# Yan-Xia/Text2Loc

Measured on AMD Instinct MI355X. Metric: coarse-retrieval queries/sec over 11k-cell DB, embed_dim=256; top-1/3/5 recall parity, higher is better.
Workload: dtype f16; 1 GPU; KITTI360Pose-sized val DB: N=11259 cells x D=256 resident in HBM, Q=4096 precomputed text embeddings per step, top-10 (float64-exact ids); n_cells=11259, embed_dim=256, top_k=10, parallelism=single-gpu, layout=one resident DB, two launches per step (scan, re-rank)

## Files before the change

include/t2l.h:

```cpp
#ifndef T2L_H_
#define T2L_H_

#include <stdint.h>

#ifdef __cplusplus
extern "C" {
#endif

#define T2L_ABI_VERSION 2
#define T2L_EMBED_DIM 256
#define T2L_OBJECT_SIZE 28
#define T2L_MAX_LOSS_BATCH 1024
#define T2L_MAX_TOPK 26

enum {
  T2L_OK = 0,
  T2L_EINVAL = -1,
  T2L_ESTATE = -2,
  T2L_EHIP = -3,
  T2L_ENOMEM = -4
};

typedef struct t2l_ctx t2l_ctx;

// ... 65 lines not shown
                       double* out_score, void* stream);

int t2l_merge_topk(t2l_ctx* ctx, const int32_t* idx, const double* score, int32_t parts, int32_t n_queries,
                   int32_t k, int32_t* out_idx, double* out_score, void* stream);

int t2l_pack_pairs(t2l_ctx* ctx, const int32_t* idx, const double* score, int32_t n_queries, int32_t k, double* pairs,
                   void* stream);
int t2l_merge_pairs(t2l_ctx* ctx, const double* pairs, int32_t parts, int32_t n_queries, int32_t k, int32_t* out_idx,
                    double* out_score, void* stream);
int t2l_merge_gathered(t2l_ctx* ctx, const void* blocks, int64_t block_bytes, int64_t score_offset, int32_t parts,
                       int32_t n_queries, int32_t k, int32_t* out_idx, double* out_score, void* stream);

int t2l_search_fallbacks(t2l_ctx* ctx, int32_t* out_count);
int t2l_search_rescored(t2l_ctx* ctx, int32_t* out_count);
int t2l_search_counters(t2l_ctx* ctx, int32_t* out8);

int t2l_contrastive_loss(t2l_ctx* ctx, const float* anchor, const float* positive, int32_t batch,
                         float temperature, float* loss, float* grad_anchor, float* grad_positive,
                         void* stream);

int t2l_text_head_load_weights(t2l_ctx* ctx, const t2l_weight_desc* w, int32_t n, const char* prefix);
int t2l_text_head_load_weights_heads(t2l_ctx* ctx, const t2l_weight_desc* w, int32_t n, const char* prefix, int32_t inter_num_heads);
int t2l_text_head(t2l_ctx* ctx, const float* hidden, int32_t n_sentences, int32_t n_tokens, float* out, int32_t* overflow,
                  void* stream);
int t2l_text_inter(t2l_ctx* ctx, const float* sent, int32_t n_descriptions, int32_t n_sentences_per, float* out, int32_t* overflow,
                   void* stream);

int t2l_fine_load_weights(t2l_ctx* ctx, const t2l_weight_desc* w, int32_t n, const t2l_model_config* cfg);

int t2l_fine_encode_objects(t2l_ctx* ctx, const t2l_packed_cells* in, float* out_desc, void* stream);
// ... 60 lines not shown
```

text2loc_amd/csrc/capi.hip:

```cpp
#include <limits.h>
#include <string.h>

#include "t2l_internal.h"

namespace t2l {

int fail(t2l_ctx* ctx, int code, const std::string& msg) {
  if (ctx) ctx->err = msg;
  return code;
}

void event_begin(t2l_ctx* ctx, const char* name, hipStream_t s) {
  if (!ctx->profile_events) return;
  EventRing& e = ctx->events[name];
  if (e.a.empty()) {
    e.a.resize(kEventRing);
    e.b.resize(kEventRing);
    for (int i = 0; i < kEventRing; ++i) {
      (void)hipEventCreate(&e.a[i]);
      (void)hipEventCreate(&e.b[i]);
    }
  }
  e.open = (e.calls++ % ctx->profile_events) == 0;
  if (e.open) (void)hipEventRecord(e.a[e.head], s);
// ... 280 lines not shown
}

int t2l_merge_gathered(t2l_ctx* ctx, const void* blocks, int64_t block_bytes, int64_t score_offset, int32_t parts, int32_t n_queries,
                       int32_t k, int32_t* out_idx, double* out_score, void* stream) {
  if (!ctx) return T2L_EINVAL;
  if (parts < 1 || n_queries < 0 || k < 1 || k > T2L_MAX_TOPK)
    return fail(ctx, T2L_EINVAL, "t2l_merge_gathered: bad parts / n_queries / k");
  if (n_queries == 0) return T2L_OK;
  if (!blocks || !out_idx) return fail(ctx, T2L_EINVAL, "t2l_merge_gathered: null buffer");
  if (reinterpret_cast<uintptr_t>(blocks) % 8)
    return fail(ctx, T2L_EINVAL, "t2l_merge_gathered: blocks must start on an 8-byte boundary");
  T2L_HIP(ctx, hipSetDevice(ctx->device));
  return merge_gathered_impl(ctx, blocks, block_bytes, score_offset, parts, n_queries, k, out_idx, out_score, (hipStream_t)stream);
}

static hipError_t read_counters(t2l_ctx* ctx, int32_t* out8) {
  if (ctx->last_search_small) {
    for (int i = 0; i < 8; ++i) out8[i] = 0;
    return hipSuccess;
  }
  hipError_t e = hipMemcpy(out8, ctx->fb_count, 8 * sizeof(int32_t), hipMemcpyDeviceToHost);
  if (e != hipSuccess || ctx->n_lanes <= 1) return e;
  for (int i = 0; i < 8; ++i) out8[i] = 0;
  for (int l = 0; l < ctx->n_lanes; ++l) {
    if (!ctx->lanes[l].ready) continue;
    int32_t c[8];
    if ((e = hipMemcpy(c, ctx->lanes[l].fb_count, sizeof(c), hipMemcpyDeviceToHost)) != hipSuccess) return e;
    for (int i = 0; i < 8; ++i) out8[i] += c[i];
  }
  return hipSuccess;
}

int t2l_search_fallbacks(t2l_ctx* ctx, int32_t* out_count) {
  if (!ctx || !out_count) return T2L_EINVAL;
  T2L_HIP(ctx, hipSetDevice(ctx->device));
  T2L_HIP(ctx, hipDeviceSynchronize());
  int32_t c[8];
  T2L_HIP(ctx, read_counters(ctx, c));
  *out_count = c[kCntExactScan] + (c[kCntExactServed] - c[kCntExactUncert]);
  return T2L_OK;
}

#ifdef T2L_STAMPS
int t2l_debug_stamps(t2l_ctx* ctx, long long* out24) {
  T2L_HIP(ctx, hipDeviceSynchronize());
  T2L_HIP(ctx, hipMemcpy(out24, ctx->fb_count + 16, 24 * sizeof(long long), hipMemcpyDeviceToHost));
  const long long init[8] = {0, 0, 0, 0, LLONG_MAX, 0, LLONG_MAX, 0};
  T2L_HIP(ctx, hipMemcpy(ctx->fb_count + 16, init, sizeof(init), hipMemcpyHostToDevice));
  return T2L_OK;
}
#endif

int t2l_search_counters(t2l_ctx* ctx, int32_t* out8) {
  if (!ctx || !out8) return T2L_EINVAL;
  T2L_HIP(ctx, hipSetDevice(ctx->device));
  T2L_HIP(ctx, hipDeviceSynchronize());
  T2L_HIP(ctx, read_counters(ctx, out8));
  return T2L_OK;
}

int t2l_search_rescored(t2l_ctx* ctx, int32_t* out_count) {
  if (!ctx || !out_count) return T2L_EINVAL;
  T2L_HIP(ctx, hipSetDevice(ctx->device));
  T2L_HIP(ctx, hipDeviceSynchronize());
  int32_t c[8];
  T2L_HIP(ctx, read_counters(ctx, c));
  *out_count = c[kCntRescored];
  return T2L_OK;
}

int t2l_contrastive_loss(t2l_ctx* ctx, const float* anchor, const float* positive, int32_t batch, float temperature,
                         float* loss, float* grad_anchor, float* grad_positive, void* stream) {
// ... 227 lines not shown
    ctx->knobs.wide_repair = (int)value;
  } else if (!strcmp(name, "search_tile_sel")) {
    ctx->knobs.search_tile_sel = value != 0;
  } else if (!strcmp(name, "search_epilogue")) {
    if (value != 0 && value != 1) return fail(ctx, T2L_EINVAL, "search_epilogue: 0 (round 6's epilogue and record layout) or 1 (default)");
    ctx->knobs.search_epilogue = (int)value;
  } else if (!strcmp(name, "search_rerank_form")) {
#ifdef T2L_RERANK_PARTS
    if (value == 2 || value == 3) {
      ctx->knobs.rerank_form = (int)value;
      return T2L_OK;
    }
#endif
    if (value != 0 && value != 1) return fail(ctx, T2L_EINVAL, "search_rerank_form: 0 (round 7's re-rank of merged records) or 1 (default: row-local merge, one gather round trip)");
    ctx->knobs.rerank_form = (int)value;
  } else if (!strcmp(name, "search_pair_ll")) {
    if (value != 5 && value != 6) return fail(ctx, T2L_EINVAL, "search_pair_ll must be 5 or 6");
    ctx->knobs.pair_ll = (int)value;
  } else if (!strcmp(name, "train_gemm_block")) {
    if (value != 0 && value != 32 && value != 64) return fail(ctx, T2L_EINVAL, "train_gemm_block must be 0 (auto), 32 or 64");
    ctx->train_gemm_block = (int)value;
  } else if (!strcmp(name, "train_bf16")) {
    if (value != 0 && value != 1 && value != 2) return fail(ctx, T2L_EINVAL, "train_bf16: 0 (f32 MFMA), 1 (bf16 operands) or 2 (split-bf16, three products)");
    ctx->train_bf16 = (int)value;
  } else if (!strcmp(name, "train_keep_adam_state")) {
    ctx->train_keep_adam = value != 0;
  } else if (!strcmp(name, "profile_rerank")) {
    ctx->knobs.profile_rerank = value != 0;
  } else if (!strcmp(name, "stats_reset")) {
    for (auto& kv : ctx->events) {
// ... 81 lines not shown
```

text2loc_amd/csrc/search.hip:

```cpp
#include <float.h>
#include <limits.h>

#include <type_traits>
#include <utility>

#include "t2l_internal.h"
#include "search_dev.h"

namespace t2l {

__device__ __forceinline__ void reset_counts(int32_t* fb_count, int32_t* fb_prev, int zero_counts, int tid) {
  if (zero_counts && tid < kCntCleared) {
    fb_count[kReportBase + tid] = fb_prev[tid];
    fb_prev[tid] = 0;
  }
  if (!zero_counts && tid == 0) {
    fb_count[kCntDeferredSegs] += fb_count[kCntDeferred];
    fb_count[kCntDeferred] = fb_count[kCntExactUncert] = 0;
  }
}


__global__ __launch_bounds__(256) void split_db_kernel(const float* __restrict__ db, uint4* __restrict__ out, int rows) {
  const int gid = blockIdx.x * 256 + threadIdx.x;
// ... 251 lines not shown
  const float* q;
  int Q, K, parts, code_bits;
  const float* cand;
  int row_offset;
  float eps_rel;
  const float* db_norm_max;
  int half_mode;
  int32_t* out_idx;
  double* out_score;
  int32_t* flags;
  int32_t* fb_count;
  float eps_rel_probe, pinf;
  int n_rows, defer, wide_cap;
  int rec6;
  int slot_bits = 0;
};

#ifndef T2L_SEL_RD
#define T2L_SEL_RD 2
#endif
template <int LL, int NS, bool MERGE = false, int SEL = 0>
__global__ __launch_bounds__(512, 1) void scanp_kernel(const uint4* __restrict__ dbt, int n_rows, int n_tiles, int code_bits,
                                                       const float* __restrict__ q, int Q, int nsplit,
                                                       float* __restrict__ cand, int32_t* __restrict__ fb_count, int32_t* __restrict__ fb_prev,
                                                       int zero_counts, float pinf, unsigned long long* __restrict__ span,
                                                       unsigned span_seq, int xcd_qgroups, int slot_bits) {
  static_assert(NS == 4, "the step loop below is unrolled for a ring of 4 slots");
  constexpr bool EPI = SEL == 1;
  static_assert(!MERGE || LL == 6, "the in-workgroup list merge is written for lists of 6");
  static_assert(!SEL || MERGE, "the tile-local selection's dropped-bound leaves through the merged record's bound");
// ... 336 lines not shown
    put_list(qrow1, w.ls1);
  }
  if (span && threadIdx.x == 0) {
    const unsigned long long t1 = __builtin_amdgcn_s_memrealtime(), tag = (unsigned long long)span_seq << 40, tm = (1ull << 40) - 1;
    *reinterpret_cast<ulonglong2*>(span + 2 * blockIdx.x) = make_ulonglong2(tag | (wg_t0 & tm), tag | (t1 & tm));
  }
  T2L_STAMP(3);
}

template <int NW>
struct WgExactSharedN {
  double score[NW][32];
  int row[NW][32];
};
typedef WgExactSharedN<4> WgExactShared;

__device__ __forceinline__ void top32_insert(double& ts, int& tr, double cd, int cr, int lane) {
  {
    const unsigned long long b31 = __double_as_longlong(ts);
    const double s31 = __longlong_as_double(((unsigned long long)__builtin_amdgcn_readlane((unsigned)(b31 >> 32), 31) << 32) |
                                            (unsigned)__builtin_amdgcn_readlane((unsigned)b31, 31));
    const int r31 = __builtin_amdgcn_readlane(tr, 31);
    if (s31 > cd || (s31 == cd && r31 <= cr)) return;
  }
  if (__ballot(lane < 32 && tr == cr) != 0ull) return;
  const unsigned long long ahead = __ballot(lane < 32 && (ts > cd || (ts == cd && tr < cr)));
  const int pos = __popcll(ahead);
  if (pos >= 32) return;
  const double up_s = __shfl_up(ts, 1);
  const int up_r = __shfl_up(tr, 1);
  if (lane == pos) {
    ts = cd;
    tr = cr;
  } else if (lane > pos && lane < 32) {
    ts = up_s;
    tr = up_r;
  }
}

template <int NW = 4>
__device__ __forceinline__ void wg_exact_scan(const float* __restrict__ db, int n_rows, const float* __restrict__ qrow, int K,
                                              int row_offset, int32_t* __restrict__ out_idx, double* __restrict__ out_score,
                                              WgExactSharedN<NW>& sh) {
  const int lane = threadIdx.x & 63, wave = threadIdx.x >> 6;
  const int seg = lane & 15, grp = lane >> 4;
  double qd[16];
  {
    const float4* qp = reinterpret_cast<const float4*>(qrow) + seg;
#pragma unroll
    for (int i = 0; i < 4; ++i) {
      const float4 v = qp[16 * i];
      qd[4 * i] = (double)v.x;
      qd[4 * i + 1] = (double)v.y;
      qd[4 * i + 2] = (double)v.z;
      qd[4 * i + 3] = (double)v.w;
    }
  }
  double my_s = -__builtin_inf();
  int my_r = INT_MAX;
  const int n_groups = (n_rows + 3) / 4;
  for (int g = wave; g < n_groups; g += NW) {
    const int row = 4 * g + grp;
    const float4* rp = reinterpret_cast<const float4*>(db + (size_t)min(row, n_rows - 1) * kD) + seg;
    double d0 = 0.0, d1 = 0.0;
#pragma unroll
    for (int i = 0; i < 4; ++i) {
      const float4 rv = rp[16 * i];
      d0 += (double)rv.x * qd[4 * i];
      d1 += (double)rv.y * qd[4 * i + 1];
      d0 += (double)rv.z * qd[4 * i + 2];
      d1 += (double)rv.w * qd[4 * i + 3];
    }
    const double d = row16_sum_f64(d0 + d1);
#pragma unroll
    for (int c = 0; c < 4; ++c) {
      const double cd = __shfl(d, 16 * c);
      const int cr = 4 * g + c;
      if (cr >= n_rows) break;
      const unsigned long long ahead = __ballot(lane < 32 && (my_s > cd || (my_s == cd && my_r < cr)));
      const int pos = __popcll(ahead);
      if (pos >= 32) continue;
      const double up_s = __shfl_up(my_s, 1);
      const int up_r = __shfl_up(my_r, 1);
      if (lane == pos) {
        my_s = cd;
        my_r = cr;
      } else if (lane > pos && lane < 32) {
        my_s = up_s;
        my_r = up_r;
      }
    }
  }
  if (lane < 32) {
    sh.score[wave][lane] = my_s;
    sh.row[wave][lane] = my_r;
  }
  __syncthreads();
  if (wave == 0) {
    constexpr int PER = NW / 2, TOT = 32 * NW;
    double sv[PER];
    int rv[PER], kv[PER];
#pragma unroll
    for (int e = 0; e < PER; ++e) {
      sv[e] = (&sh.score[0][0])[64 * e + lane];
      rv[e] = (&sh.row[0][0])[64 * e + lane];
      kv[e] = 0;
    }
    for (int o = 0; o < TOT; ++o) {
      const double os = (&sh.score[0][0])[o];
      const int orow = (&sh.row[0][0])[o];
#pragma unroll
      for (int e = 0; e < PER; ++e) kv[e] += (os > sv[e] || (os == sv[e] && orow < rv[e])) ? 1 : 0;
    }
    if (lane < K) {
      out_idx[lane] = -1;
      if (out_score) out_score[lane] = -__builtin_inf();
    }
#pragma unroll
    for (int e = 0; e < PER; ++e)
      if (rv[e] != INT_MAX && kv[e] < K) {
        out_idx[kv[e]] = rv[e] + row_offset;
        if (out_score) out_score[kv[e]] = sv[e];
      }
  }
  __syncthreads();
}


__device__ __forceinline__ void publish_report(int32_t* fb_count, int32_t* host_stat, int seq) {
  if (host_stat && seq > 0) {
    const int32_t* prev = fb_count + kReportBase;
    host_stat[kStatFlagged] = prev[kCntStatMode] == 2 ? prev[kCntProbe] : prev[kCntUnsettled];
    host_stat[kStatTotal] = prev[kCntQ];
    host_stat[kStatExact] = prev[kCntExactScan] + prev[kCntDeferred] + prev[kCntDeferredSegs];
    host_stat[kStatMode] = prev[kCntStatMode];
    host_stat[kStatRescored] = prev[kCntStatMode] == 2 ? prev[kCntProbe] : prev[kCntRescored];
    __hip_atomic_store(&host_stat[kStatSeq], seq, __ATOMIC_RELEASE, __HIP_MEMORY_SCOPE_SYSTEM);
  }
}

#ifdef T2L_STAMPS
constexpr int kRrStampWaves = 4096, kRrStampSlots = 8;
__device__ long long g_rr_stamps[kRrStampWaves * kRrStampSlots];
#define T2L_RR_STAMP(k, dep)                                                                \
  {                                                                                         \
    __builtin_amdgcn_sched_barrier(0);                                                      \
    asm volatile("" ::"v"(dep));                                                            \
    const long long t_ = __builtin_amdgcn_s_memrealtime();                                  \
    if (lane == 0 && qid < kRrStampWaves) g_rr_stamps[qid * kRrStampSlots + (k)] = t_;      \
    __builtin_amdgcn_sched_barrier(0);                                                      \
  }
#else
#define T2L_RR_STAMP(k, dep)
#endif

template <int LL, int L, bool MG = false, int FORM = 0>
__device__ __forceinline__ void rerank_query(const RerankArgs& a, const int qid, const int lane, int* my_wg_flag, int* wr_buf) {
  static_assert(!MG || LL == kMergedLL, "merged records are 8 floats");
  static_assert(FORM == 0 || (MG && L == 16), "the row-local form is written for merged records, 16 candidates");
  constexpr bool RLM = FORM == 1 || FORM == 2;
  constexpr bool RLG = FORM == 1 || FORM == 3;
  constexpr int kKeys = RLM ? LL - 2 : LL;
  const float* __restrict__ db = a.db;
  const float* __restrict__ q = a.q;
  const int Q = a.Q, K = a.K, parts = a.parts, code_bits = a.code_bits, row_offset = a.row_offset, half_mode = a.half_mode;
  const int slack_bits = MG ? code_bits + 2 : code_bits;
  const int strided_rows = half_mode ? a.n_rows : 0;
  auto krow = [&](float key, int part) {
    if constexpr (MG) {
      const int b = __float_as_int(key), src = b & 3;
      return key_row(__int_as_float(b >> 2), 2 * (part + (src >> 1) * parts) + (src & 1), 2 * parts, code_bits, strided_rows);
    } else {
      return key_row(key, part, parts >> 1, code_bits, strided_rows);
    }
  };
  const float* __restrict__ cand = a.cand;
  const float eps_rel = a.eps_rel, eps_rel_probe = a.eps_rel_probe, pinf = a.pinf;
  const float* __restrict__ db_norm_max = a.db_norm_max;
  int32_t* __restrict__ out_idx = a.out_idx;
  double* __restrict__ out_score = a.out_score;
  int32_t* __restrict__ flags = a.flags;
  int32_t* __restrict__ fb_count = a.fb_count;
  const int n_rows = a.n_rows, defer = a.defer, wide_cap = a.wide_cap;

  float lst[LL];
  {
// ... 465 lines not shown
          for (int c = 0; c < 4; ++c) {
            const double cd = __shfl(d, 16 * c);
            const int cr = __shfl(row_c, 16 * c);
            if (cr != INT_MAX) top32_insert(ts, tr, cd, cr, lane);
          }
#pragma unroll
          for (int i = 0; i < 4; ++i) cur[i] = nxt[i];
          row_c = row_n;
        }
        if (lane < K) {
          out_idx[(size_t)qid * K + lane] = tr == INT_MAX ? -1 : tr + row_offset;
          if (out_score) out_score[(size_t)qid * K + lane] = ts;
        }
        if (lane == 0) atomicAdd(&fb_count[kCntWideRepair], 1);
        settled = true;
      }
    }
  }
  if (lane == 0) {
    const int flag = !representable ? 2 : ((certified || settled) ? 0 : 1);
    flags[qid] = flag;
    if (!certified || !representable) atomicAdd(&fb_count[kCntRescored], 1);
    if (flag) {
      atomicAdd(&fb_count[kCntUnsettled], 1);
      if (!defer) *my_wg_flag = flag;
      else if (flag == 2) flags[4 * Q + atomicAdd(&fb_count[kCntExactUncert], 1)] = qid;
      else flags[3 * Q + atomicAdd(&fb_count[kCntDeferred], 1)] = qid;
    }
  }
  }
  }
}

template <int LL, int L, bool MG = false, int FORM = 0>
__global__ __launch_bounds__(256, (MG ? 4 : 1)) void rerank_kernel(const float* __restrict__ db, const float* __restrict__ q, int Q,
                                                     int K, int parts, int code_bits,
                                                     const float* __restrict__ cand, int row_offset, float eps_rel,
                                                     const float* __restrict__ db_norm_max, int half_mode,
                                                     int32_t* __restrict__ out_idx, double* __restrict__ out_score,
                                                     int32_t* __restrict__ flags, int32_t* __restrict__ fb_count,
                                                     float eps_rel_probe, float pinf, int n_rows, int defer, int stat_mode,
                                                     int32_t* __restrict__ host_stat, int seq, int wide_cap, int rec6, int slot_bits) {
  __shared__ WgExactShared exact_sh;
  __shared__ int wg_flag[4];
  __shared__ int wide_rows[4][kWideCap];
  const RerankArgs a{db, q, Q, K, parts, code_bits, cand, row_offset, eps_rel, db_norm_max, half_mode, out_idx, out_score, flags, fb_count,
                     eps_rel_probe, pinf, n_rows, defer, wide_cap, rec6, slot_bits};
  const int lane = threadIdx.x & 63;
  const int qid = blockIdx.x * 4 + (threadIdx.x >> 6);
  if (threadIdx.x < 4) wg_flag[threadIdx.x] = 0;
  if (blockIdx.x == 0 && threadIdx.x == 0) {
    publish_report(fb_count, host_stat, seq);
    fb_count[kCntQ] = Q;
    fb_count[kCntStatMode] = stat_mode;
  }
  __syncthreads();
#ifdef T2L_STAMPS
  if (qid < Q && qid < kRrStampWaves && lane == 0) {
    long long* st = g_rr_stamps + qid * kRrStampSlots;
    st[0] = __builtin_amdgcn_s_memrealtime();
    st[5] = 0;
    st[7] = (long long)(unsigned)__builtin_amdgcn_s_getreg((31 << 11) | 4) |
            ((long long)(unsigned)__builtin_amdgcn_s_getreg((31 << 11) | 20) << 32);
  }
#endif
  if (qid < Q) rerank_query<LL, L, MG, FORM>(a, qid, lane, &wg_flag[threadIdx.x >> 6], wide_rows[threadIdx.x >> 6]);
  T2L_RR_STAMP(6, lane);
  __syncthreads();
#pragma unroll 1
  for (int w = 0; w < 4; ++w) {
    if (!wg_flag[w]) continue;
    const int fq = blockIdx.x * 4 + w;
    if (threadIdx.x == 0) atomicAdd(&fb_count[kCntExactScan], 1);
    wg_exact_scan(db, n_rows, q + (size_t)fq * kD, K, row_offset, out_idx + (size_t)fq * K,
                  out_score ? out_score + (size_t)fq * K : nullptr, exact_sh);
  }
}

__global__ __launch_bounds__(256) void db_norm_kernel(const float* __restrict__ db, int n_rows, float* out) {
  __shared__ float red[4];
  __shared__ int red_a[4];
  const int lane = threadIdx.x & 63, wave = threadIdx.x >> 6;
  float m = 0.f;
  int am = 0;
  for (int row = blockIdx.x * 4 + wave; row < n_rows; row += gridDim.x * 4) {
    const float4 v = reinterpret_cast<const float4*>(db + (size_t)row * kD)[lane];
    float s = v.x * v.x + v.y * v.y + v.z * v.z + v.w * v.w;
    int a = max(max(__float_as_int(v.x) & 0x7fffffff, __float_as_int(v.y) & 0x7fffffff),
                max(__float_as_int(v.z) & 0x7fffffff, __float_as_int(v.w) & 0x7fffffff));
#pragma unroll
// ... 133 lines not shown
      else
        hipLaunchKernelGGL((scanw_kernel<LL, 4>), grid, block, p.lds, s, dbs, n_rows, p.n_tiles, p.code_bits, q, Q, p.scan_nsplit,
                           ctx->cand_score, ctx->fb_count, ctx->fb_prev, zero, __builtin_inff());
      event_end(ctx, "search_scan", s);
    };
    switch (p.LL) {
      case 8: launch(std::integral_constant<int, 8>{}); break;
      case 16: launch(std::integral_constant<int, 16>{}); break;
      default: launch(std::integral_constant<int, 32>{}); break;
    }
  }
  T2L_HIP(ctx, hipGetLastError());
  auto rerank = [&](auto kern) {
    launch_timed(ctx, "search_rerank", p.time_rerank, kern, dim3((Q + 3) / 4), dim3(256), 0, s, db, q, Q, K, p.rerank_parts, p.code_bits,
                 ctx->cand_score, row_offset, p.eps_rel, ctx->db_norm_max, p.half_mode, out_idx, out_score, ctx->flags, ctx->fb_count,
                 p.eps_probe, __builtin_inff(), n_rows, p.defer, p.stat_mode, ctx->host_stat_dev, seq, p.wide_cap, p.rec6, p.rerank_slot_bits);
  };
  switch (p.rerank) {
    case RerankKernel::kLists5: rerank(&rerank_kernel<5, 16>); break;
    case RerankKernel::kLists6: rerank(&rerank_kernel<6, 16>); break;
    case RerankKernel::kLists8: rerank(&rerank_kernel<8, 16>); break;
    case RerankKernel::kLists16: rerank(&rerank_kernel<16, 16>); break;
    case RerankKernel::kLists32: rerank(&rerank_kernel<32, 32>); break;
    case RerankKernel::kRecords:
      if (p.rerank_form == 1) rerank(&rerank_kernel<kMergedLL, 16, true, 1>);
#ifdef T2L_RERANK_PARTS
      else if (p.rerank_form == 2) rerank(&rerank_kernel<kMergedLL, 16, true, 2>);
      else if (p.rerank_form == 3) rerank(&rerank_kernel<kMergedLL, 16, true, 3>);
#endif
      else rerank(&rerank_kernel<kMergedLL, 16, true>);
      break;
// ... 168 lines not shown
```

text2loc_amd/csrc/search_plan.h:

```cpp
#pragma once
#include <stddef.h>
#include <stdint.h>

namespace t2l {

constexpr int kScanDim = 256;
constexpr int kTileRows = 32;
constexpr int kRowStrideF = kScanDim + 4;
constexpr int kTileFloats = kTileRows * kRowStrideF;
constexpr int kHalfTileBytes = kTileRows * 512;
constexpr int kMaxParts = 64;
constexpr int kMaxPerTiles = 512;
constexpr int kSegmentRows = (kMaxParts / 2) * kMaxPerTiles * 32;
constexpr int kWideQPerWave = 64;
constexpr int kWideQPerBlock = 4 * kWideQPerWave;
constexpr int kMergedLL = 8;
constexpr int kWideCap = 1024;

struct SearchKnobs {
  double eps_scale = 1.0;
  int nsplit_override = 0;
  int search_mode = 0;
  int pair_ll = 6;
  int search_epilogue = 1;
  int search_tile_sel = 1;
  int wide_repair = 512;
  int search_merge = 2;
  int xcd_qgroups = 4;
  int profile_rerank = 1;
  int rerank_form = 1;
};

enum ReportField {
  kStatSeq = 0,
  kStatFlagged = 1,
  kStatTotal = 2,
  kStatExact = 3,
  kStatMode = 4,
  kStatRescored = 5,
  kStatInts = 8,
};

struct SearchPolicy {
  bool escalated = false;
  bool heavy = false;
// ... 76 lines not shown
};

struct SegmentPlan {
  int L, n_tiles, nsplit, per, code_bits, LL;
  bool pair;
  size_t cand_bytes;
  ScanKernel scan;
  unsigned grid, block;
  size_t lds;
  int scan_nsplit;
  int xq, slot_bits;
  bool merged;
  float eps_rel, eps_probe;
  int half_mode, stat_mode, defer;
  RerankKernel rerank;
  int rerank_parts, rec6, rerank_slot_bits, wide_cap;
  bool time_rerank;
  int rerank_form;
};

inline SegmentPlan plan_segment(const SearchKnobs& k, int eff_mode, bool merge_live, bool heavy, int Q, int K, int rows) {
  SegmentPlan p{};
  const int qpb = kWideQPerBlock;
  const int n_qblocks = (Q + qpb - 1) / qpb;
  const int L = (K <= 10) ? 16 : 32;
  const int n_tiles = ((rows > 0 ? rows : 0) + kTileRows - 1) / kTileRows;
  auto imax = [](int a, int b) { return a > b ? a : b; };
  auto imin = [](int a, int b) { return a < b ? a : b; };
  const bool pair_ok = eff_mode == 0 && L == 16 && n_tiles >= 16 && Q >= 256;
  int nsplit = k.nsplit_override;
  if (nsplit <= 0) {
// ... 20 lines not shown
  p.nsplit = nsplit;
  p.pair = pair;
  p.per = per;
  p.code_bits = code_bits;
  p.LL = LL;
  p.cand_bytes = (size_t)n_qblocks * qpb * 2 * nsplit * LL * sizeof(float);

  p.half_mode = eff_mode == 0;
  const bool probing = k.search_mode == 0 && eff_mode == 2;
  const double operand_eps = eff_mode == 0 ? 9.85e-4 : (eff_mode == 2 ? 2.0e-5 : 0.0);
  p.eps_rel = (float)(k.eps_scale * ((kScanDim + 8) * 5.9604644775390625e-08 + operand_eps));
  p.eps_probe = probing ? (float)(k.eps_scale * ((kScanDim + 8) * 5.9604644775390625e-08 + 9.85e-4)) : 0.f;
  p.stat_mode = probing ? 2 : (p.half_mode ? 1 : 0);
  p.defer = heavy ? 1 : 0;
  p.wide_cap = imin(k.wide_repair, kWideCap);
  p.time_rerank = k.profile_rerank != 0;
  p.xq = 1;
  if (pair) {
    p.scan_nsplit = nsplit / 2;
    p.grid = (unsigned)(n_qblocks * (nsplit / 2));
    p.block = 512;
    p.lds = (size_t)4 * 2 * kHalfTileBytes + (size_t)256 * (kMergedLL + 3) * sizeof(float);
    int xq = k.xcd_qgroups;
    {
      const int nqb = n_qblocks, ns = nsplit / 2;
      if (xq < 2 || 8 % xq || nqb % xq || ns % (8 / xq) || (nqb * ns) % 8) xq = 1;
    }
    int slot_bits = 0;
    if (k.search_epilogue && xq > 1)
      for (int gs = 8 / xq; gs > 1; gs >>= 1) ++slot_bits;
// ... 28 lines not shown
```

text2loc_amd/csrc/t2l_internal.h:

```cpp
#pragma once
#include <hip/hip_runtime.h>

#include <atomic>
#include <hip/hip_ext.h>
#include <stdint.h>

#include <string>
#include <unordered_map>
#include <vector>

#include "t2l.h"
#include "search_plan.h"
#include "text_inter_plan.h"

namespace t2l {

constexpr int kD = T2L_EMBED_DIM;
constexpr int kS = T2L_OBJECT_SIZE;
constexpr int kSP = 32;

static_assert(kScanDim == kD, "search_plan.h plans for rows of kD floats");
constexpr int kQPerWave = 32;
constexpr int kScanWaves = 4;
constexpr int kQPerBlock = kQPerWave * kScanWaves;
constexpr int kStageCap = 32;

enum CounterSlot {
  kCntExactScan = 0,
  kCntRescored = 1,
  kCntUnsettled = 2,
  kCntProbe = 3,
  kCntDeferred = 4,
  kCntWideRepair = 5,
  kCntExactUncert = 6,
  kCntExactServed = 7,
  kCntQ = 9,
  kCntStatMode = 10,
  kCntDeferredSegs = 12,
  kCntCleared = 16,
  kReportBase = 64,
  kBankInts = 128,
};

constexpr int kEventRing = 512;
constexpr int kSpanRing = 64;
constexpr int kSpanWgs = 512;
struct EventRing {
  std::vector<hipEvent_t> a, b;
  int head = 0;
  int count = 0;
// ... 194 lines not shown
```

text2loc_amd/engine.py:

```python
from __future__ import annotations

import ctypes as C
import os
import os.path as osp
from typing import Dict, Optional, Tuple

import numpy as np
import torch

EMBED_DIM = 256
OBJECT_SIZE = 28
COMPILED_EMBED_DIMS = (128, 256)
COMPILED_HEAD_DIMS = (32, 64)
MAX_OBJECT_SIZE = 32
COMPILED_SHAPES = ("coarse_embed_dim in {128, 256}; object_inter_module_num_heads with head_dim 32 or 64 (2 or 4 heads at 128, 4 or 8 at "
                   "256); object_size 1..32; object_inter_module_num_layers 1..4")
MAX_TOPK = 26
_LIB_PATH = os.environ.get("T2L_LIB") or osp.join(osp.dirname(osp.abspath(__file__)), "libt2l.so")


class T2LError(RuntimeError):
    pass


# ... 54 lines not shown
    "t2l_db_rows": (C.c_int64, [C.c_void_p]),
    "t2l_search": (C.c_int, [C.c_void_p, C.c_void_p, C.c_int32, C.c_int32, C.c_void_p, C.c_void_p, C.c_void_p]),
    "t2l_search_join": (C.c_int, [C.c_void_p, C.c_void_p]),
    "t2l_search_many": (C.c_int, [C.c_void_p, C.c_void_p, C.c_int32, C.c_int32, C.c_int32, C.c_void_p, C.c_void_p, C.c_void_p]),
    "t2l_search_ordered": (C.c_int, [C.c_void_p, C.c_void_p, C.c_int32, C.c_int32, C.c_void_p, C.c_void_p, C.c_void_p]),
    "t2l_merge_topk": (C.c_int, [C.c_void_p, C.c_void_p, C.c_void_p, C.c_int32, C.c_int32, C.c_int32, C.c_void_p,
                                 C.c_void_p, C.c_void_p]),
    "t2l_pack_pairs": (C.c_int, [C.c_void_p, C.c_void_p, C.c_void_p, C.c_int32, C.c_int32, C.c_void_p, C.c_void_p]),
    "t2l_merge_pairs": (C.c_int, [C.c_void_p, C.c_void_p, C.c_int32, C.c_int32, C.c_int32, C.c_void_p, C.c_void_p,
                                  C.c_void_p]),
    "t2l_merge_gathered": (C.c_int, [C.c_void_p, C.c_void_p, C.c_int64, C.c_int64, C.c_int32, C.c_int32, C.c_int32, C.c_void_p, C.c_void_p,
                                     C.c_void_p]),
    "t2l_search_fallbacks": (C.c_int, [C.c_void_p, C.POINTER(C.c_int32)]),
    "t2l_search_rescored": (C.c_int, [C.c_void_p, C.POINTER(C.c_int32)]),
    "t2l_search_counters": (C.c_int, [C.c_void_p, C.POINTER(C.c_int32)]),
    "t2l_contrastive_loss": (C.c_int, [C.c_void_p, C.c_void_p, C.c_void_p, C.c_int32, C.c_float, C.c_void_p,
                                       C.c_void_p, C.c_void_p, C.c_void_p]),
    "t2l_text_head_load_weights": (C.c_int, [C.c_void_p, C.POINTER(_WeightDesc), C.c_int32, C.c_char_p]),
    "t2l_text_head_load_weights_heads": (C.c_int, [C.c_void_p, C.POINTER(_WeightDesc), C.c_int32, C.c_char_p, C.c_int32]),
    "t2l_text_head": (C.c_int, [C.c_void_p, C.c_void_p, C.c_int32, C.c_int32, C.c_void_p, C.c_void_p, C.c_void_p]),
    "t2l_text_inter": (C.c_int, [C.c_void_p, C.c_void_p, C.c_int32, C.c_int32, C.c_void_p, C.c_void_p, C.c_void_p]),
    "t2l_fine_load_weights": (C.c_int, [C.c_void_p, C.POINTER(_WeightDesc), C.c_int32, C.POINTER(_ModelConfig)]),
    "t2l_fine_encode_objects": (C.c_int, [C.c_void_p, C.POINTER(_PackedCells), C.c_void_p, C.c_void_p]),
    "t2l_fine_match": (C.c_int, [C.c_void_p, C.c_void_p, C.c_void_p, C.c_void_p, C.c_void_p, C.c_int32, C.c_int32, C.c_void_p,
                                 C.c_void_p]),
    "t2l_train_bind": (C.c_int, [C.c_void_p, C.POINTER(_TrainTensor), C.c_int32, C.POINTER(_ModelConfig)]),
    "t2l_encode_cells_train": (C.c_int, [C.c_void_p, C.POINTER(_PackedCells), C.c_float, C.c_uint32, C.c_void_p, C.c_void_p]),
    "t2l_encode_cells_backward": (C.c_int, [C.c_void_p, C.c_void_p, C.c_void_p, C.c_void_p]),
    "t2l_fine_train_bind": (C.c_int, [C.c_void_p, C.POINTER(_TrainTensor), C.c_int32, C.POINTER(_ModelConfig)]),
    "t2l_fine_train_forward": (C.c_int, [C.c_void_p, C.POINTER(_PackedCells), C.c_void_p, C.c_void_p, C.c_int32, C.c_int32, C.c_float,
# ... 588 lines not shown
                   torch.empty((nb, Q, k), dtype=torch.float64, device=queries.device))
        self._check(self.lib.t2l_search_many(self._h, self._ptr(queries, torch.float32, "queries"), nb, Q, int(k), out[0].data_ptr(),
                                             out[1].data_ptr(), _stream_ptr(self.device)))
        return out

    def search_fallbacks(self) -> int:
        c = C.c_int32(0)
        self._check(self.lib.t2l_search_fallbacks(self._h, C.byref(c)))
        return int(c.value)

    def search_counters(self) -> dict:
        c = (C.c_int32 * 8)()
        self._check(self.lib.t2l_search_counters(self._h, c))
        names = ("valu_exact_scans", "rescored", "to_fallback_kernel", "probe", "deferred_to_mfma_exact", "wide_repairs",
                 "mfma_exact_uncertified", "mfma_exact_served")
        return {n: int(c[i]) for i, n in enumerate(names)}

    def search_rescored(self) -> int:
        c = C.c_int32(0)
        self._check(self.lib.t2l_search_rescored(self._h, C.byref(c)))
        return int(c.value)

    def contrastive_loss(self, anchor: torch.Tensor, positive: torch.Tensor, temperature: float, need_grad=True):
        B = int(anchor.shape[0])
        loss = torch.empty((1,), dtype=torch.float32, device=anchor.device)
        ga = torch.empty_like(anchor) if need_grad else None
        gp = torch.empty_like(positive) if need_grad else None
        self._check(self.lib.t2l_contrastive_loss(
            self._h, self._ptr(anchor, torch.float32, "anchor"), self._ptr(positive, torch.float32, "positive"), B,
            float(temperature), loss.data_ptr(), self._ptr(ga, torch.float32, "ga"), self._ptr(gp, torch.float32, "gp"),
            _stream_ptr(self.device)))
# ... 10 lines not shown
```

Before: 106.3 million queries/s.

## Re-score only surviving candidate rows in the workgroup exact fallback stage

When a query is unsettled, the workgroup exact stage now re-scores only the candidate rows whose keys clear a per-query threshold, plus fully rescanning tiles from bad partitions, instead of scanning the whole shard. The per-wave handoff flag becomes a struct carrying the threshold and masks. Row scoring gets a three-deep register prefetch ring, and the merge step adds duplicate removal. The aim is to cut the full-DB f64 scan cost for fallback queries, at the price of extra bookkeeping and added correctness risk in the candidate list construction.

```diff
diff --git a/include/t2l.h b/include/t2l.h
--- a/include/t2l.h
+++ b/include/t2l.h
@@ -103,6 +103,7 @@
 int t2l_search_fallbacks(t2l_ctx* ctx, int32_t* out_count);
 int t2l_search_rescored(t2l_ctx* ctx, int32_t* out_count);
 int t2l_search_counters(t2l_ctx* ctx, int32_t* out8);
+int t2l_search_partial_rescores(t2l_ctx* ctx, int32_t* out_count);
 
 int t2l_contrastive_loss(t2l_ctx* ctx, const float* anchor, const float* positive, int32_t batch,
                          float temperature, float* loss, float* grad_anchor, float* grad_positive,
diff --git a/text2loc_amd/csrc/capi.hip b/text2loc_amd/csrc/capi.hip
--- a/text2loc_amd/csrc/capi.hip
+++ b/text2loc_amd/csrc/capi.hip
@@ -318,19 +318,19 @@
   return merge_gathered_impl(ctx, blocks, block_bytes, score_offset, parts, n_queries, k, out_idx, out_score, (hipStream_t)stream);
 }
 
-static hipError_t read_counters(t2l_ctx* ctx, int32_t* out8) {
+static hipError_t read_counters(t2l_ctx* ctx, int32_t* out, int n = 8) {
   if (ctx->last_search_small) {
-    for (int i = 0; i < 8; ++i) out8[i] = 0;
+    for (int i = 0; i < n; ++i) out[i] = 0;
     return hipSuccess;
   }
-  hipError_t e = hipMemcpy(out8, ctx->fb_count, 8 * sizeof(int32_t), hipMemcpyDeviceToHost);
+  hipError_t e = hipMemcpy(out, ctx->fb_count, n * sizeof(int32_t), hipMemcpyDeviceToHost);
   if (e != hipSuccess || ctx->n_lanes <= 1) return e;
-  for (int i = 0; i < 8; ++i) out8[i] = 0;
+  for (int i = 0; i < n; ++i) out[i] = 0;
   for (int l = 0; l < ctx->n_lanes; ++l) {
     if (!ctx->lanes[l].ready) continue;
-    int32_t c[8];
-    if ((e = hipMemcpy(c, ctx->lanes[l].fb_count, sizeof(c), hipMemcpyDeviceToHost)) != hipSuccess) return e;
-    for (int i = 0; i < 8; ++i) out8[i] += c[i];
+    int32_t c[kCntWgPartial + 1];
+    if ((e = hipMemcpy(c, ctx->lanes[l].fb_count, n * sizeof(int32_t), hipMemcpyDeviceToHost)) != hipSuccess) return e;
+    for (int i = 0; i < n; ++i) out[i] += c[i];
   }
   return hipSuccess;
 }
@@ -360,6 +360,16 @@
   T2L_HIP(ctx, hipSetDevice(ctx->device));
   T2L_HIP(ctx, hipDeviceSynchronize());
   T2L_HIP(ctx, read_counters(ctx, out8));
+  return T2L_OK;
+}
+
+int t2l_search_partial_rescores(t2l_ctx* ctx, int32_t* out_count) {
+  if (!ctx || !out_count) return T2L_EINVAL;
+  T2L_HIP(ctx, hipSetDevice(ctx->device));
+  T2L_HIP(ctx, hipDeviceSynchronize());
+  int32_t c[kCntWgPartial + 1];
+  T2L_HIP(ctx, read_counters(ctx, c, kCntWgPartial + 1));
+  *out_count = c[kCntWgPartial];
   return T2L_OK;
 }
 
@@ -617,6 +627,9 @@
 #endif
     if (value != 0 && value != 1) return fail(ctx, T2L_EINVAL, "search_rerank_form: 0 (round 7's re-rank of merged records) or 1 (default: row-local merge, one gather round trip)");
     ctx->knobs.rerank_form = (int)value;
+  } else if (!strcmp(name, "search_wg_partial")) {
+    if (value != 0 && value != 1) return fail(ctx, T2L_EINVAL, "search_wg_partial: 1 (default: the workgroup stage re-scores the rows that can still matter) or 0 (it scans the whole shard)");
+    ctx->knobs.wg_partial = (int)value;
   } else if (!strcmp(name, "search_pair_ll")) {
     if (value != 5 && value != 6) return fail(ctx, T2L_EINVAL, "search_pair_ll must be 5 or 6");
     ctx->knobs.pair_ll = (int)value;
diff --git a/text2loc_amd/csrc/search.hip b/text2loc_amd/csrc/search.hip
--- a/text2loc_amd/csrc/search.hip
+++ b/text2loc_amd/csrc/search.hip
@@ -289,6 +289,7 @@
   int n_rows, defer, wide_cap;
   int rec6;
   int slot_bits = 0;
+  int wg_partial = 0;
 };
 
 #ifndef T2L_SEL_RD
@@ -655,6 +656,13 @@
   int row[NW][32];
 };
 typedef WgExactSharedN<4> WgExactShared;
+constexpr int kWgRing = 3;
+
+struct WgHandoff {
+  int flag, partial;
+  float thr;
+  unsigned long long bad_mask, d_mask;
+};
 
 __device__ __forceinline__ void top32_insert(double& ts, int& tr, double cd, int cr, int lane) {
   {
@@ -679,59 +687,61 @@
   }
 }
 
-template <int NW = 4>
-__device__ __forceinline__ void wg_exact_scan(const float* __restrict__ db, int n_rows, const float* __restrict__ qrow, int K,
-                                              int row_offset, int32_t* __restrict__ out_idx, double* __restrict__ out_score,
-                                              WgExactSharedN<NW>& sh) {
-  const int lane = threadIdx.x & 63, wave = threadIdx.x >> 6;
-  const int seg = lane & 15, grp = lane >> 4;
-  double qd[16];
-  {
-    const float4* qp = reinterpret_cast<const float4*>(qrow) + seg;
+__device__ __forceinline__ void wg_load_query(const float* __restrict__ qrow, int seg, float4 (&qf)[4]) {
+  const float4* qp = reinterpret_cast<const float4*>(qrow) + seg;
+#pragma unroll
+  for (int i = 0; i < 4; ++i) qf[i] = qp[16 * i];
+}
+
+template <int NW, class RowOf>
+__device__ __forceinline__ void wg_score_groups(int tid, const float* __restrict__ db, const float4 (&qf)[4], int n_groups, RowOf row_of,
+                                                double& ts, int& tr) {
+  const int lane = tid & 63, wave = tid >> 6, seg = lane & 15;
+  float4 ring[kWgRing][4];
+  int ring_row[kWgRing];
+  auto fetch = [&](auto s_tag, int g) {
+    constexpr int s = decltype(s_tag)::value;
+    const int row = g < n_groups ? row_of(g) : INT_MAX;
+    ring_row[s] = row;
+    const float4* rp = reinterpret_cast<const float4*>(db + (size_t)(row == INT_MAX ? 0 : row) * kD) + seg;
+#pragma unroll
+    for (int i = 0; i < 4; ++i) ring[s][i] = rp[16 * i];
+  };
+  auto stage = [&](auto s_tag, int g) {
+    constexpr int s = decltype(s_tag)::value;
+    double d0 = 0.0, d1 = 0.0;
 #pragma unroll
     for (int i = 0; i < 4; ++i) {
-      const float4 v = qp[16 * i];
-      qd[4 * i] = (double)v.x;
-      qd[4 * i + 1] = (double)v.y;
-      qd[4 * i + 2] = (double)v.z;
-      qd[4 * i + 3] = (double)v.w;
-    }
-  }
-  double my_s = -__builtin_inf();
-  int my_r = INT_MAX;
-  const int n_groups = (n_rows + 3) / 4;
-  for (int g = wave; g < n_groups; g += NW) {
-    const int row = 4 * g + grp;
-    const float4* rp = reinterpret_cast<const float4*>(db + (size_t)min(row, n_rows - 1) * kD) + seg;
-    double d0 = 0.0, d1 = 0.0;
-#pragma unroll
-    for (int i = 0; i < 4; ++i) {
-      const float4 rv = rp[16 * i];
-      d0 += (double)rv.x * qd[4 * i];
-      d1 += (double)rv.y * qd[4 * i + 1];
-      d0 += (double)rv.z * qd[4 * i + 2];
-      d1 += (double)rv.w * qd[4 * i + 3];
+      float4 qv = qf[i];
+      asm volatile("" : "+v"(qv.x), "+v"(qv.y), "+v"(qv.z), "+v"(qv.w));
+      d0 += (double)ring[s][i].x * (double)qv.x;
+      d1 += (double)ring[s][i].y * (double)qv.y;
+      d0 += (double)ring[s][i].z * (double)qv.z;
+      d1 += (double)ring[s][i].w * (double)qv.w;
+      __builtin_amdgcn_sched_barrier(0);
     }
     const double d = row16_sum_f64(d0 + d1);
+    const int row_c = ring_row[s];
+    fetch(s_tag, g + kWgRing * NW);
 #pragma unroll
     for (int c = 0; c < 4; ++c) {
       const double cd = __shfl(d, 16 * c);
-      const int cr = 4 * g + c;
-      if (cr >= n_rows) break;
-      const unsigned long long ahead = __ballot(lane < 32 && (my_s > cd || (my_s == cd && my_r < cr)));
-      const int pos = __popcll(ahead);
-      if (pos >= 32) continue;
-      const double up_s = __shfl_up(my_s, 1);
-      const int up_r = __shfl_up(my_r, 1);
-      if (lane == pos) {
-        my_s = cd;
-        my_r = cr;
-      } else if (lane > pos && lane < 32) {
-        my_s = up_s;
-        my_r = up_r;
-      }
-    }
-  }
+      const int cr = __shfl(row_c, 16 * c);
+      if (cr != INT_MAX) top32_insert(ts, tr, cd, cr, lane);
+    }
+  };
+  auto prime = [&](auto s_tag) { fetch(s_tag, wave + decltype(s_tag)::value * NW); };
+  const_for<0>(prime, std::make_integer_sequence<int, kWgRing>{});
+  for (int g0 = wave; g0 < n_groups; g0 += kWgRing * NW) {
+    auto turn = [&](auto s_tag) { stage(s_tag, g0 + decltype(s_tag)::value * NW); };
+    const_for<0>(turn, std::make_integer_sequence<int, kWgRing>{});
+  }
+}
+
+template <int NW>
+__device__ __forceinline__ void wg_merge_top(int tid, double my_s, int my_r, int K, int row_offset, int32_t* __restrict__ out_idx,
+                                             double* __restrict__ out_score, WgExactSharedN<NW>& sh) {
+  const int lane = tid & 63, wave = tid >> 6;
   if (lane < 32) {
     sh.score[wave][lane] = my_s;
     sh.row[wave][lane] = my_r;
@@ -741,12 +751,28 @@
     constexpr int PER = NW / 2, TOT = 32 * NW;
     double sv[PER];
     int rv[PER], kv[PER];
+    bool dup[PER];
 #pragma unroll
     for (int e = 0; e < PER; ++e) {
       sv[e] = (&sh.score[0][0])[64 * e + lane];
       rv[e] = (&sh.row[0][0])[64 * e + lane];
       kv[e] = 0;
-    }
+      dup[e] = false;
+    }
+    for (int o = 0; o < TOT; ++o) {
+      const int orow = (&sh.row[0][0])[o];
+#pragma unroll
+      for (int e = 0; e < PER; ++e) dup[e] = dup[e] || (o < 64 * e + lane && orow == rv[e]);
+    }
+#pragma unroll
+    for (int e = 0; e < PER; ++e)
+      if (dup[e] && rv[e] != INT_MAX) {
+        sv[e] = -__builtin_inf();
+        rv[e] = INT_MAX;
+        (&sh.score[0][0])[64 * e + lane] = sv[e];
+        (&sh.row[0][0])[64 * e + lane] = rv[e];
+      }
+    __builtin_amdgcn_fence(__ATOMIC_SEQ_CST, "workgroup");
     for (int o = 0; o < TOT; ++o) {
       const double os = (&sh.score[0][0])[o];
       const int orow = (&sh.row[0][0])[o];
@@ -767,6 +793,79 @@
   __syncthreads();
 }
 
+__device__ __forceinline__ int record_key_row(float key, int part, int parts, int code_bits, int strided_rows) {
+  const int b = __float_as_int(key), src = b & 3;
+  return key_row(__int_as_float(b >> 2), 2 * (part + (src >> 1) * parts) + (src & 1), 2 * parts, code_bits, strided_rows);
+}
+
+template <bool MG, int NW = 4>
+__device__ __forceinline__ void wg_exact_rank(const RerankArgs& a, int fq, const bool partial, const WgHandoff& ho, int* list, int* n_list,
+                                              WgExactSharedN<NW>& sh) {
+  int tid = threadIdx.x;
+  asm volatile("" : "+v"(tid));
+  const int lane = tid & 63, wave = tid >> 6, grp = lane >> 4;
+  const int parts = a.parts, code_bits = a.code_bits, n_rows = a.n_rows, strided_rows = a.half_mode ? a.n_rows : 0;
+  auto krow = [&](float key, int part) {
+    const int row = record_key_row(key, part, parts, code_bits, strided_rows);
+    return (unsigned)row < (unsigned)n_rows ? row : INT_MAX;
+  };
+  float4 qf[4];
+  wg_load_query(a.q + (size_t)fq * kD, lane & 15, qf);
+  unsigned long long bad_left = 0ull;
+  int n_groups = (n_rows + 3) / 4;
+  if (MG && partial) {
+    const float thr = ho.thr;
+    const unsigned long long bad_mask = ho.bad_mask, d_mask = ho.d_mask;
+    if (wave == 0) {
+      const int part = min(lane, parts - 1);
+      const float4* mine = reinterpret_cast<const float4*>(a.cand + ((size_t)fq * parts + record_slot(part, parts, a.slot_bits)) * kMergedLL);
+      const float4 v0 = mine[0], v1 = mine[1];
+      const float key[kMergedLL - 1] = {v0.x, v0.y, v0.z, v0.w, v1.x, v1.y, v1.z};
+      const bool good = lane < parts && ((bad_mask >> lane) & 1ull) == 0ull;
+      const int n_keys = a.rec6 ? kMergedLL - 2 : kMergedLL - 1;
+      const unsigned long long lt_mask = (1ull << lane) - 1ull;
+      int base = 0;
+#pragma unroll
+      for (int i = 0; i < kMergedLL - 1; ++i) {
+        const bool pred = good && i < n_keys && key[i] != T2L_NEG_INF && key[i] >= thr;
+        const unsigned long long m = __ballot(pred);
+        if (pred) list[base + __popcll(m & lt_mask)] = krow(key[i], lane);
+        base += __popcll(m);
+      }
+      for (unsigned long long m = d_mask; m != 0ull; m &= m - 1ull) {
+        const int b = __ffsll((long long)m) - 1;
+        const int kb = __shfl(__float_as_int(key[kMergedLL - 2]), b);
+        if (lane < kTileSelGroup) list[base + lane] = krow(__int_as_float((kb & ~((kTileSelGroup - 1) << 2)) | (lane << 2)), b);
+        base += kTileSelGroup;
+      }
+      if (lane < 4) list[base + lane] = INT_MAX;
+      if (lane == 0) *n_list = base;
+    }
+    __syncthreads();
+    bad_left = bad_mask;
+    n_groups = (*n_list + 3) >> 2;
+  }
+  double my_s = -__builtin_inf();
+  int my_r = INT_MAX;
+  const int n_tiles = (n_rows + kTileRows - 1) / kTileRows;
+  int b = -1;
+#pragma unroll 1
+  for (;;) {
+    wg_score_groups<NW>(tid, a.db, qf, n_groups, [&](int g) {
+      const int idx = 4 * g + grp;
+      if constexpr (MG) {
+        if (b >= 0) return krow(__int_as_float(idx), b);
+        if (partial) return list[idx];
+      }
+      return idx < n_rows ? idx : INT_MAX;
+    }, my_s, my_r);
+    if (bad_left == 0ull) break;
+    b = __ffsll((long long)bad_left) - 1;
+    bad_left &= bad_left - 1ull;
+    n_groups = (b < parts && b < n_tiles) ? 16 * ((n_tiles - b + 2 * parts - 1) / (2 * parts)) : 0;
+  }
+  wg_merge_top<NW>(tid, my_s, my_r, a.K, a.row_offset, a.out_idx + (size_t)fq * a.K, a.out_score ? a.out_score + (size_t)fq * a.K : nullptr, sh);
+}
 
 __device__ __forceinline__ void publish_report(int32_t* fb_count, int32_t* host_stat, int seq) {
   if (host_stat && seq > 0) {
@@ -796,7 +895,7 @@
 #endif
 
 template <int LL, int L, bool MG = false, int FORM = 0>
-__device__ __forceinline__ void rerank_query(const RerankArgs& a, const int qid, const int lane, int* my_wg_flag, int* wr_buf) {
+__device__ __forceinline__ void rerank_query(const RerankArgs& a, const int qid, const int lane, WgHandoff* my_wg, int* wr_buf) {
   static_assert(!MG || LL == kMergedLL, "merged records are 8 floats");
   static_assert(FORM == 0 || (MG && L == 16), "the row-local form is written for merged records, 16 candidates");
   constexpr bool RLM = FORM == 1 || FORM == 2;
@@ -809,8 +908,7 @@
   const int strided_rows = half_mode ? a.n_rows : 0;
   auto krow = [&](float key, int part) {
     if constexpr (MG) {
-      const int b = __float_as_int(key), src = b & 3;
-      return key_row(__int_as_float(b >> 2), 2 * (part + (src >> 1) * parts) + (src & 1), 2 * parts, code_bits, strided_rows);
+      return record_key_row(key, part, parts, code_bits, strided_rows);
     } else {
       return key_row(key, part, parts >> 1, code_bits, strided_rows);
     }
@@ -1306,6 +1404,11 @@
         }
         if (lane == 0) atomicAdd(&fb_count[kCntWideRepair], 1);
         settled = true;
+      } else if (MG && a.wg_partial && !defer && lane == 0) {
+        my_wg->thr = thr;
+        my_wg->bad_mask = bad_mask;
+        my_wg->d_mask = d_mask;
+        my_wg->partial = 1;
       }
     }
   }
@@ -1315,7 +1418,7 @@
     if (!certified || !representable) atomicAdd(&fb_count[kCntRescored], 1);
     if (flag) {
       atomicAdd(&fb_count[kCntUnsettled], 1);
-      if (!defer) *my_wg_flag = flag;
+      if (!defer) my_wg->flag = flag;
       else if (flag == 2) flags[4 * Q + atomicAdd(&fb_count[kCntExactUncert], 1)] = qid;
       else flags[3 * Q + atomicAdd(&fb_count[kCntDeferred], 1)] = qid;
     }
@@ -1332,15 +1435,16 @@
                                                      int32_t* __restrict__ out_idx, double* __restrict__ out_score,
                                                      int32_t* __restrict__ flags, int32_t* __restrict__ fb_count,
                                                      float eps_rel_probe, float pinf, int n_rows, int defer, int stat_mode,
-                                                     int32_t* __restrict__ host_stat, int seq, int wide_cap, int rec6, int slot_bits) {
+                                                     int32_t* __restrict__ host_stat, int seq, int wide_cap, int rec6, int slot_bits, int wg_partial) {
   __shared__ WgExactShared exact_sh;
-  __shared__ int wg_flag[4];
+  __shared__ WgHandoff wg_ho[4];
+  __shared__ int wg_n_list;
   __shared__ int wide_rows[4][kWideCap];
   const RerankArgs a{db, q, Q, K, parts, code_bits, cand, row_offset, eps_rel, db_norm_max, half_mode, out_idx, out_score, flags, fb_count,
-                     eps_rel_probe, pinf, n_rows, defer, wide_cap, rec6, slot_bits};
+                     eps_rel_probe, pinf, n_rows, defer, wide_cap, rec6, slot_bits, wg_partial};
   const int lane = threadIdx.x & 63;
   const int qid = blockIdx.x * 4 + (threadIdx.x >> 6);
-  if (threadIdx.x < 4) wg_flag[threadIdx.x] = 0;
+  if (threadIdx.x < 4) wg_ho[threadIdx.x].flag = wg_ho[threadIdx.x].partial = 0;
   if (blockIdx.x == 0 && threadIdx.x == 0) {
     publish_report(fb_count, host_stat, seq);
     fb_count[kCntQ] = Q;
@@ -1356,16 +1460,21 @@
             ((long long)(unsigned)__builtin_amdgcn_s_getreg((31 << 11) | 20) << 32);
   }
 #endif
-  if (qid < Q) rerank_query<LL, L, MG, FORM>(a, qid, lane, &wg_flag[threadIdx.x >> 6], wide_rows[threadIdx.x >> 6]);
+  const int wv = __builtin_amdgcn_readfirstlane(threadIdx.x >> 6);
+  if (qid < Q) rerank_query<LL, L, MG, FORM>(a, qid, lane, &wg_ho[wv], wide_rows[wv]);
   T2L_RR_STAMP(6, lane);
   __syncthreads();
 #pragma unroll 1
   for (int w = 0; w < 4; ++w) {
-    if (!wg_flag[w]) continue;
+    const int flag = wg_ho[w].flag;
+    if (!flag) continue;
     const int fq = blockIdx.x * 4 + w;
-    if (threadIdx.x == 0) atomicAdd(&fb_count[kCntExactScan], 1);
-    wg_exact_scan(db, n_rows, q + (size_t)fq * kD, K, row_offset, out_idx + (size_t)fq * K,
-                  out_score ? out_score + (size_t)fq * K : nullptr, exact_sh);
+    const bool partial = MG && flag == 1 && wg_ho[w].partial;
+    if (threadIdx.x == 0) {
+      atomicAdd(&fb_count[kCntExactScan], 1);
+      if (partial) atomicAdd(&fb_count[kCntWgPartial], 1);
+    }
+    wg_exact_rank<MG>(a, fq, partial, wg_ho[w], wide_rows[0], &wg_n_list, exact_sh);
   }
 }
 
@@ -1529,7 +1638,7 @@
   auto rerank = [&](auto kern) {
     launch_timed(ctx, "search_rerank", p.time_rerank, kern, dim3((Q + 3) / 4), dim3(256), 0, s, db, q, Q, K, p.rerank_parts, p.code_bits,
                  ctx->cand_score, row_offset, p.eps_rel, ctx->db_norm_max, p.half_mode, out_idx, out_score, ctx->flags, ctx->fb_count,
-                 p.eps_probe, __builtin_inff(), n_rows, p.defer, p.stat_mode, ctx->host_stat_dev, seq, p.wide_cap, p.rec6, p.rerank_slot_bits);
+                 p.eps_probe, __builtin_inff(), n_rows, p.defer, p.stat_mode, ctx->host_stat_dev, seq, p.wide_cap, p.rec6, p.rerank_slot_bits, p.wg_partial);
   };
   switch (p.rerank) {
     case RerankKernel::kLists5: rerank(&rerank_kernel<5, 16>); break;
diff --git a/text2loc_amd/csrc/search_plan.h b/text2loc_amd/csrc/search_plan.h
--- a/text2loc_amd/csrc/search_plan.h
+++ b/text2loc_amd/csrc/search_plan.h
@@ -29,6 +29,7 @@
   int xcd_qgroups = 4;
   int profile_rerank = 1;
   int rerank_form = 1;
+  int wg_partial = 1;
 };
 
 enum ReportField {
@@ -135,7 +136,7 @@
   float eps_rel, eps_probe;
   int half_mode, stat_mode, defer;
   RerankKernel rerank;
-  int rerank_parts, rec6, rerank_slot_bits, wide_cap;
+  int rerank_parts, rec6, rerank_slot_bits, wide_cap, wg_partial;
   bool time_rerank;
   int rerank_form;
 };
@@ -186,6 +187,7 @@
   p.stat_mode = probing ? 2 : (p.half_mode ? 1 : 0);
   p.defer = heavy ? 1 : 0;
   p.wide_cap = imin(k.wide_repair, kWideCap);
+  p.wg_partial = k.wg_partial ? 1 : 0;
   p.time_rerank = k.profile_rerank != 0;
   p.xq = 1;
   if (pair) {
diff --git a/text2loc_amd/csrc/t2l_internal.h b/text2loc_amd/csrc/t2l_internal.h
--- a/text2loc_amd/csrc/t2l_internal.h
+++ b/text2loc_amd/csrc/t2l_internal.h
@@ -34,6 +34,7 @@
   kCntWideRepair = 5,
   kCntExactUncert = 6,
   kCntExactServed = 7,
+  kCntWgPartial = 8,
   kCntQ = 9,
   kCntStatMode = 10,
   kCntDeferredSegs = 12,
diff --git a/text2loc_amd/engine.py b/text2loc_amd/engine.py
--- a/text2loc_amd/engine.py
+++ b/text2loc_amd/engine.py
@@ -92,6 +92,7 @@
     "t2l_search_fallbacks": (C.c_int, [C.c_void_p, C.POINTER(C.c_int32)]),
     "t2l_search_rescored": (C.c_int, [C.c_void_p, C.POINTER(C.c_int32)]),
     "t2l_search_counters": (C.c_int, [C.c_void_p, C.POINTER(C.c_int32)]),
+    "t2l_search_partial_rescores": (C.c_int, [C.c_void_p, C.POINTER(C.c_int32)]),
     "t2l_contrastive_loss": (C.c_int, [C.c_void_p, C.c_void_p, C.c_void_p, C.c_int32, C.c_float, C.c_void_p,
                                        C.c_void_p, C.c_void_p, C.c_void_p]),
     "t2l_text_head_load_weights": (C.c_int, [C.c_void_p, C.POINTER(_WeightDesc), C.c_int32, C.c_char_p]),
@@ -710,7 +711,11 @@
         self._check(self.lib.t2l_search_counters(self._h, c))
         names = ("valu_exact_scans", "rescored", "to_fallback_kernel", "probe", "deferred_to_mfma_exact", "wide_repairs",
                  "mfma_exact_uncertified", "mfma_exact_served")
-        return {n: int(c[i]) for i, n in enumerate(names)}
+        out = {n: int(c[i]) for i, n in enumerate(names)}
+        p = C.c_int32(0)
+        self._check(self.lib.t2l_search_partial_rescores(self._h, C.byref(p)))
+        out["wg_partial_rescores"] = int(p.value)
+        return out
 
     def search_rescored(self) -> int:
         c = C.c_int32(0)
```

Result: no change. 105.2 million queries/s (-1.0%).
